# lbarseghyan/diffusion-models

Hardware: AMD Instinct MI355X
Metric: sampled images/sec, 32x32 U-Net (dim 64, mults 1-2-4-8), DDPM-1000 (higher is better)
Workload: dtype f32; 1 GPU; ddpm1000_32x32_unet64_b256_per_gpu; sampler=p_sample_loop (DDPM), sampler_steps=1000, batch_per_gpu=256, global_batch=256, hip_graph=True, graph_captures=1, parallelism=batch-shard x1, one all-gather per sample()

## Files before the change

### diffusion-models_amd/csrc/linattn_fused.hip

```cpp
#include "conv_device.h"

#include <cmath>
#include <vector>

namespace dm {

static constexpr int LA_DH = 32;
static constexpr int LA_HEADS = 4;
static constexpr int LA_HID = LA_DH * LA_HEADS;
static constexpr int LA_CTX = LA_DH * LA_DH + LA_DH;
static constexpr int LA_TOK1 = 128;
__host__ __device__ constexpr int la_tok1(int C) { return C <= 64 ? 256 : LA_TOK1; }
static constexpr int LA_TOK2 = 64;
static constexpr int LA_TOKI = 128;

__host__ __device__ static inline int la_row_of(int e, int half) { return (e & 3) + 8 * (e >> 2) + 4 * half; }

bool linattn_fused_eligible(int C, int heads, int dh) {
    static const bool off = env_flag("DM_NO_FUSED_LINATTN");
    return !off && heads == LA_HEADS && dh == LA_DH && (C == 64 || C == 128);
}

bool linattn_fused_pack(const float* w_qkv, const float* norm_g, const float* w_out, const float* mem_kv, int C,
                        std::vector<float>& wq, std::vector<float>& wk, std::vector<float>& wv, std::vector<float>& wo,
                        std::vector<float>& kbound) {
    const int G = C / 8;
    const float sq = std::sqrt((float)C);
    auto pack_proj = [&](int which, std::vector<float>& dst) {
        dst.assign((size_t)LA_HEADS * G * 64 * 4, 0.f);
        for (int h = 0; h < LA_HEADS; ++h)
            for (int g = 0; g < G; ++g)
                for (int lane = 0; lane < 64; ++lane)
                    for (int s = 0; s < 4; ++s) {
                        const int l = lane & 31, half = lane >> 5;
                        const int row = which * LA_HID + h * LA_DH + l, c = 8 * g + 4 * half + s;
                        dst[(((size_t)h * G + g) * 64 + lane) * 4 + s] = w_qkv[(size_t)row * C + c] * (norm_g[c] * sq);
                    }
    };
    pack_proj(0, wq);
    pack_proj(1, wk);
    pack_proj(2, wv);
    wo.clear();
    (void)w_out;
    kbound.assign(LA_HID, 0.f);
    bool ok = true;
    for (int h = 0; h < LA_HEADS; ++h)
        for (int d = 0; d < LA_DH; ++d) {
            double ss = 0;
            for (int c = 0; c < C; ++c) {
                const double v = (double)w_qkv[(size_t)(LA_HID + h * LA_DH + d) * C + c] * norm_g[c] * sq;
                ss += v * v;
            }
            float bnd = (float)(std::sqrt(ss) * 1.0001);
            for (int j = 0; j < 4; ++j) bnd = std::fmax(bnd, mem_kv[((size_t)h * LA_DH + d) * 4 + j]);
            kbound[h * LA_DH + d] = bnd;
            if (!(bnd < 40.f)) ok = false;
        }
    return ok;
}

size_t linattn_fused_ws_floats(int B, int n) {
    const int nblk = (n + LA_TOK1 - 1) / LA_TOK1;
    return (size_t)B * nblk * LA_HEADS * LA_CTX + (size_t)B * LA_HEADS * 128 * LA_DH;
}

template <int C, int TOK>
__device__ __forceinline__ void la_stage_rows(const float* __restrict__ xb, int nt, float* xs, float* rn) {
    constexpr int XS = C + 4, Q = C / 4;
    const int tid = threadIdx.x;
#pragma unroll
    for (int i = 0; i < TOK * Q / 256; ++i) {
        const int it = tid + 256 * i;
        const int row = it / Q, q = it - row * Q;
        f32x4 v = make_f32x4(0.f, 0.f, 0.f, 0.f);
        if (row < nt) v = *reinterpret_cast<const f32x4*>(xb + (size_t)row * C + 4 * q);
        *reinterpret_cast<f32x4*>(xs + row * XS + 4 * q) = v;
    }
    __syncthreads();
    if (tid < TOK) {
        float ss = 0.f;
#pragma unroll
        for (int q = 0; q < Q; ++q) {
            const f32x4 v = *reinterpret_cast<const f32x4*>(xs + tid * XS + 4 * q);
            ss += v.x * v.x + v.y * v.y + v.z * v.z + v.w * v.w;
        }
        rn[tid] = 1.0f / fmaxf(sqrtf(ss), 1e-12f);
    }
}

template <int C, int TOK>
__global__ __launch_bounds__(256) void linattn_ctx_fused_kernel(const float* __restrict__ x, const LinAttnFused w,
                                                                float* __restrict__ ws, int n, int nblk) {
    constexpr int G = C / 8, XS = C + 4;
    extern __shared__ __attribute__((aligned(16))) float smem[];
    float* xs = smem;
    float* rn = smem + TOK * XS;
    const int blk = blockIdx.x, b = blockIdx.y;
    const int tid = threadIdx.x, lane = tid & 63, h = tid >> 6;
    const int l31 = lane & 31, lh = lane >> 5;
    const int t0 = blk * TOK;
    const int nt = min(TOK, n - t0);

    f32x4 wk[G], wv[G];
#pragma unroll
    for (int g = 0; g < G; ++g) {
        wk[g] = *reinterpret_cast<const f32x4*>(w.wk + (((size_t)h * G + g) * 64 + lane) * 4);
        wv[g] = *reinterpret_cast<const f32x4*>(w.wv + (((size_t)h * G + g) * 64 + lane) * 4);
    }
    const float kb = w.kbound[h * LA_DH + l31];
    la_stage_rows<C, TOK>(x + ((size_t)b * n + t0) * C, nt, xs, rn);
    __syncthreads();

    f32x16 cacc;
#pragma unroll
    for (int e = 0; e < 16; ++e) cacc[e] = 0.f;
    float ksum = 0.f;
    if (blk == 0) {
        const float* mk = w.mem_kv + (size_t)h * LA_DH * 4;
        const float* mv = w.mem_kv + (size_t)(LA_HEADS + h) * LA_DH * 4;
#pragma unroll
        for (int j = 0; j < 4; j += 2) {
            const float a = __expf(mk[l31 * 4 + j + lh] - kb);
            ksum += a;
            cacc = __builtin_amdgcn_mfma_f32_32x32x2f32(a, mv[l31 * 4 + j + lh], cacc, 0, 0, 0);
        }
    }
    for (int st = 0; st < TOK / 32; ++st) {
        if (st * 32 >= nt) break;
        f32x16 kacc, vacc;
#pragma unroll
        for (int e = 0; e < 16; ++e) {
            kacc[e] = 0.f;
            vacc[e] = 0.f;
        }
        const float* xr = xs + (st * 32 + l31) * XS + 4 * lh;
#pragma unroll
        for (int g = 0; g < G; ++g) {
            const f32x4 a = *reinterpret_cast<const f32x4*>(xr + 8 * g);
#pragma unroll
            for (int s = 0; s < 4; ++s) {
                kacc = __builtin_amdgcn_mfma_f32_32x32x2f32(a[s], wk[g][s], kacc, 0, 0, 0);
                vacc = __builtin_amdgcn_mfma_f32_32x32x2f32(a[s], wv[g][s], vacc, 0, 0, 0);
            }
        }
#pragma unroll
        for (int m = 0; m < 4; ++m) {
            const f32x4 r4 = *reinterpret_cast<const f32x4*>(rn + st * 32 + 8 * m + 4 * lh);
#pragma unroll
            for (int i = 0; i < 4; ++i) {
                const int e = 4 * m + i;
                const bool valid = st * 32 + 8 * m + 4 * lh + i < nt;
                const float a = valid ? __expf(kacc[e] * r4[i] - kb) : 0.f;
                ksum += a;
                cacc = __builtin_amdgcn_mfma_f32_32x32x2f32(a, vacc[e] * r4[i], cacc, 0, 0, 0);
            }
        }
    }
    float* cp = ws + (((size_t)b * nblk + blk) * LA_HEADS + h) * LA_CTX;
#pragma unroll
    for (int e = 0; e < 16; ++e) cp[la_row_of(e, lh) * LA_DH + l31] = cacc[e];
    ksum += __shfl_xor(ksum, 32);
    if (lh == 0) cp[LA_DH * LA_DH + l31] = ksum;
}

template <int C>
__global__ __launch_bounds__(256) void linattn_ctx_reduce_kernel(const float* __restrict__ ws,
                                                                 const float* __restrict__ w_out,
                                                                 float* __restrict__ mz, int nblk) {
    constexpr int MT = C / 32;
    __shared__ float cs[LA_DH][LA_DH + 1];
    const int h = blockIdx.x, b = blockIdx.y;
    const int tid = threadIdx.x, lane = tid & 63, e4 = tid >> 6;
    const int l31 = lane & 31, lh = lane >> 5;
#pragma unroll
    for (int i = 0; i < 4; ++i) {
        const int d = 8 * e4 + 4 * lh + i;
        float c = 0.f, k = 0.f;
#pragma unroll 8
        for (int kb = 0; kb < nblk; ++kb) {
            const float* cp = ws + (((size_t)b * nblk + kb) * LA_HEADS + h) * LA_CTX;
            c += cp[d * LA_DH + l31];
            k += cp[LA_DH * LA_DH + d];
        }
        cs[d][l31] = c / k;
    }
    __syncthreads();
    const int mt = e4;
    if (mt < MT) {
        const float* wr = w_out + (size_t)(32 * mt + l31) * LA_HID + h * LA_DH;
        f32x16 acc;
#pragma unroll
        for (int e = 0; e < 16; ++e) acc[e] = 0.f;
#pragma unroll
        for (int st = 0; st < 16; ++st)
            acc = __builtin_amdgcn_mfma_f32_32x32x2f32(cs[l31][2 * st + lh], wr[2 * st + lh], acc, 0, 0, 0);
        float* op = mz + ((((size_t)b * LA_HEADS + h) * MT + mt) * 4) * 64 * 4 + lane * 4;
#pragma unroll
        for (int q = 0; q < 4; ++q)
            *reinterpret_cast<f32x4*>(op + q * 64 * 4) = make_f32x4(acc[4 * q], acc[4 * q + 1], acc[4 * q + 2], acc[4 * q + 3]);
    }
}

template <int C>
__device__ __forceinline__ void la_image_load(const float* __restrict__ xb, int t0, int n,
                                              f32x4 (&pre)[LA_TOKI * (C / 4) / 512]) {
    constexpr int Q = C / 4;
    const int tid = threadIdx.x;
#pragma unroll
    for (int i = 0; i < LA_TOKI * Q / 512; ++i) {
        const int it = tid + 512 * i;
        const int row = it / Q, q = it - row * Q;
        const int t = t0 + row;
        const f32x4 v = *reinterpret_cast<const f32x4*>(xb + (size_t)min(t, n - 1) * C + 4 * q);
        pre[i] = t < n ? v : make_f32x4(0.f, 0.f, 0.f, 0.f);
    }
}

template <int C>
__device__ __forceinline__ void la_image_store(const f32x4 (&pre)[LA_TOKI * (C / 4) / 512], float* xs, float* rn) {
    constexpr int XS = C + 4, Q = C / 4;
    const int tid = threadIdx.x;
#pragma unroll
    for (int i = 0; i < LA_TOKI * Q / 512; ++i) {
        const int it = tid + 512 * i;
        const int row = it / Q, q = it - row * Q;
        const f32x4 v = pre[i];
        *reinterpret_cast<f32x4*>(xs + row * XS + 4 * q) = v;
        float ss = v.x * v.x + v.y * v.y + v.z * v.z + v.w * v.w;
#pragma unroll
        for (int o = 1; o < Q; o <<= 1) ss += __shfl_xor(ss, o);
        if (q == 0) rn[row] = 1.0f / fmaxf(sqrtf(ss), 1e-12f);
    }
}

template <int C>
__global__ __launch_bounds__(512) void linattn_ctx_image_kernel(const float* __restrict__ x, const LinAttnFused w,
                                                                float* __restrict__ mz, int n) {
    constexpr int G = C / 8, XS = C + 4, CT = C / 32, TB = LA_TOKI, NP = TB * (C / 4) / 512;
    extern __shared__ __attribute__((aligned(16))) float smem[];
    float* rnb = smem + 2 * TB * XS;
    const int b = blockIdx.x;
    const int tid = threadIdx.x, lane = tid & 63, wid = tid >> 6;
    const int h = wid & 3, th = wid >> 2;
    const int l31 = lane & 31, lh = lane >> 5;
    const float* xb = x + (size_t)b * n * C;
    const int nb = (n + TB - 1) / TB;

    f32x4 wk[G];
#pragma unroll
    for (int g = 0; g < G; ++g) wk[g] = *reinterpret_cast<const f32x4*>(w.wk + (((size_t)h * G + g) * 64 + lane) * 4);
    const float kb = w.kbound[h * LA_DH + l31];

    f32x4 pre[NP];
    la_image_load<C>(xb, 0, n, pre);
    la_image_store<C>(pre, smem, rnb);
    __syncthreads();

    f32x16 pacc[CT];
#pragma unroll
    for (int ct = 0; ct < CT; ++ct)
#pragma unroll
        for (int e = 0; e < 16; ++e) pacc[ct][e] = 0.f;
    float ksum = 0.f;
    for (int blk = 0; blk < nb; ++blk) {
        const bool more = blk + 1 < nb;
        if (more) la_image_load<C>(xb, (blk + 1) * TB, n, pre);
        const float* xs = smem + (blk & 1) * TB * XS;
        const float* rn = rnb + (blk & 1) * TB;
#pragma unroll
        for (int j = 0; j < 2; ++j) {
            const int tb = 32 * (th + 2 * j);
            const int nt = n - blk * TB - tb;
            if (nt <= 0) break;
            f32x16 kacc;
#pragma unroll
            for (int e = 0; e < 16; ++e) kacc[e] = 0.f;
            const float* xr = xs + (tb + l31) * XS + 4 * lh;
#pragma unroll
            for (int g = 0; g < G; ++g) {
                const f32x4 a = *reinterpret_cast<const f32x4*>(xr + 8 * g);
#pragma unroll
                for (int s = 0; s < 4; ++s) kacc = __builtin_amdgcn_mfma_f32_32x32x2f32(a[s], wk[g][s], kacc, 0, 0, 0);
            }
            const float* xc = xs + (tb + 4 * lh) * XS + l31;
#pragma unroll
            for (int m = 0; m < 4; ++m) {
                const f32x4 r4 = *reinterpret_cast<const f32x4*>(rn + tb + 8 * m + 4 * lh);
#pragma unroll
                for (int i = 0; i < 4; ++i) {
                    const int e = 4 * m + i;
                    const bool valid = 8 * m + 4 * lh + i < nt;
                    const float a = valid ? __expf(kacc[e] * r4[i] - kb) : 0.f;
                    ksum += a;
                    const float ar = a * r4[i];
#pragma unroll
                    for (int ct = 0; ct < CT; ++ct)
                        pacc[ct] = __builtin_amdgcn_mfma_f32_32x32x2f32(xc[(8 * m + i) * XS + 32 * ct], ar, pacc[ct], 0, 0, 0);
                }
            }
        }
        if (more) la_image_store<C>(pre, smem + ((blk + 1) & 1) * TB * XS, rnb + ((blk + 1) & 1) * TB);
        __syncthreads();
    }

    float* cps = smem + (size_t)h * CT * 16 * 64 + lane;
    float* cks = smem + LA_HEADS * CT * 16 * 64 + h * 64 + lane;
    if (th == 1) {
#pragma unroll
        for (int ct = 0; ct < CT; ++ct)
#pragma unroll
            for (int e = 0; e < 16; ++e) cps[(ct * 16 + e) * 64] = pacc[ct][e];
        *cks = ksum;
    }
    __syncthreads();
    if (th == 1) return;

    ksum += *cks;
    f32x16 tacc;
#pragma unroll
    for (int e = 0; e < 16; ++e) tacc[e] = 0.f;
    {
        const float* mk = w.mem_kv + (size_t)h * LA_DH * 4;
        const float* mv = w.mem_kv + (size_t)(LA_HEADS + h) * LA_DH * 4;
#pragma unroll
        for (int j = 0; j < 4; j += 2) {
            const float a = __expf(mk[l31 * 4 + j + lh] - kb);
            ksum += a;
            tacc = __builtin_amdgcn_mfma_f32_32x32x2f32(mv[l31 * 4 + j + lh], a, tacc, 0, 0, 0);
        }
    }
#pragma unroll
    for (int ct = 0; ct < CT; ++ct)
#pragma unroll
        for (int q = 0; q < 4; ++q) {
            const f32x4 wv = *reinterpret_cast<const f32x4*>(w.wv + (((size_t)h * G + 4 * ct + q) * 64 + lane) * 4);
#pragma unroll
            for (int i = 0; i < 4; ++i) {
                const int e = 4 * q + i;
                tacc = __builtin_amdgcn_mfma_f32_32x32x2f32(wv[i], pacc[ct][e] + cps[(ct * 16 + e) * 64], tacc, 0, 0, 0);
            }
        }
    ksum += __shfl_xor(ksum, 32);
#pragma unroll
    for (int e = 0; e < 16; ++e) tacc[e] = tacc[e] / ksum;
#pragma unroll
    for (int mt = 0; mt < CT; ++mt) {
        const float* wr = w.wo_raw + (size_t)(32 * mt + l31) * LA_HID + h * LA_DH + 4 * lh;
        f32x16 macc;
#pragma unroll
        for (int e = 0; e < 16; ++e) macc[e] = 0.f;
#pragma unroll
        for (int q = 0; q < 4; ++q) {
            const f32x4 wo = *reinterpret_cast<const f32x4*>(wr + 8 * q);
#pragma unroll
            for (int i = 0; i < 4; ++i) macc = __builtin_amdgcn_mfma_f32_32x32x2f32(tacc[4 * q + i], wo[i], macc, 0, 0, 0);
        }
        float* op = mz + ((((size_t)b * LA_HEADS + h) * CT + mt) * 4) * 64 * 4 + lane * 4;
#pragma unroll
        for (int q = 0; q < 4; ++q)
            *reinterpret_cast<f32x4*>(op + q * 64 * 4) =
                make_f32x4(macc[4 * q], macc[4 * q + 1], macc[4 * q + 2], macc[4 * q + 3]);
    }
}

template <int C>
__global__ __launch_bounds__(256) void linattn_out_fused_kernel(const float* __restrict__ x, const LinAttnFused w,
                                                                const float* __restrict__ mz, float* __restrict__ y,
                                                                int n, int add_x, float scale) {
    constexpr int G = C / 8, XS = C + 4, TOK = LA_TOK2, MT = C / 32, Q = C / 4;
    extern __shared__ __attribute__((aligned(16))) float smem[];
    float* xs = smem;
    float* rn = smem + TOK * XS;
    float* zb = rn + TOK;
    const int blk = blockIdx.x, b = blockIdx.y;
    const int tid = threadIdx.x, lane = tid & 63, h = tid >> 6;
    const int l31 = lane & 31, lh = lane >> 5;
    const int t0 = blk * TOK;
    const int nt = min(TOK, n - t0);

    f32x4 wq[G];
#pragma unroll
    for (int g = 0; g < G; ++g) wq[g] = *reinterpret_cast<const f32x4*>(w.wq + (((size_t)h * G + g) * 64 + lane) * 4);
    f32x4 mreg[MT][4];
    {
        const float* mzp = mz + ((size_t)b * LA_HEADS + h) * MT * 4 * 64 * 4 + lane * 4;
#pragma unroll
        for (int mt = 0; mt < MT; ++mt)
#pragma unroll
            for (int e4 = 0; e4 < 4; ++e4) mreg[mt][e4] = *reinterpret_cast<const f32x4*>(mzp + (mt * 4 + e4) * 64 * 4);
    }
    la_stage_rows<C, TOK>(x + ((size_t)b * n + t0) * C, nt, xs, rn);
    __syncthreads();

    for (int st = 0; st < TOK / 32; ++st) {
        if (st * 32 >= nt) break;
        f32x16 qacc;
#pragma unroll
        for (int e = 0; e < 16; ++e) qacc[e] = 0.f;
        const float* xr = xs + (st * 32 + l31) * XS + 4 * lh;
#pragma unroll
        for (int g = 0; g < G; ++g) {
            const f32x4 a = *reinterpret_cast<const f32x4*>(xr + 8 * g);
#pragma unroll
            for (int s = 0; s < 4; ++s) qacc = __builtin_amdgcn_mfma_f32_32x32x2f32(wq[g][s], a[s], qacc, 0, 0, 0);
        }
        const float r = rn[st * 32 + l31];
        float m = -INFINITY;
#pragma unroll
        for (int e = 0; e < 16; ++e) {
            qacc[e] *= r;
            m = fmaxf(m, qacc[e]);
        }
        m = fmaxf(m, __shfl_xor(m, 32));
        float ssum = 0.f;
#pragma unroll
        for (int e = 0; e < 16; ++e) {
            qacc[e] = __expf(qacc[e] - m);
            ssum += qacc[e];
        }
        ssum += __shfl_xor(ssum, 32);
        const float inv = scale / ssum;
#pragma unroll
        for (int e = 0; e < 16; ++e) qacc[e] *= inv;
#pragma unroll
        for (int mt = 0; mt < MT; ++mt) {
            f32x16 zacc;
#pragma unroll
            for (int e = 0; e < 16; ++e) zacc[e] = 0.f;
#pragma unroll
            for (int e4 = 0; e4 < 4; ++e4) {
#pragma unroll
                for (int i = 0; i < 4; ++i)
                    zacc = __builtin_amdgcn_mfma_f32_32x32x2f32(mreg[mt][e4][i], qacc[4 * e4 + i], zacc, 0, 0, 0);
            }
            float* zr = zb + (h * 32 + l31) * XS + 32 * mt + 4 * lh;
#pragma unroll
            for (int m4 = 0; m4 < 4; ++m4)
                *reinterpret_cast<f32x4*>(zr + 8 * m4) =
                    make_f32x4(zacc[4 * m4], zacc[4 * m4 + 1], zacc[4 * m4 + 2], zacc[4 * m4 + 3]);
        }
        __syncthreads();
#pragma unroll
        for (int i = 0; i < 32 * Q / 256; ++i) {
            const int it = tid + 256 * i;
            const int tok = it / Q, q4 = it - tok * Q;
            f32x4 z = *reinterpret_cast<const f32x4*>(w.bias + 4 * q4);
#pragma unroll
            for (int hh = 0; hh < LA_HEADS; ++hh) z += *reinterpret_cast<const f32x4*>(zb + (hh * 32 + tok) * XS + 4 * q4);
            float ss = z.x * z.x + z.y * z.y + z.z * z.z + z.w * z.w;
#pragma unroll
            for (int o = 1; o < Q; o <<= 1) ss += __shfl_xor(ss, o);
            z = z * fast_rsq(fmaxf(ss, 1e-24f)) * *reinterpret_cast<const f32x4*>(w.og + 4 * q4);
            if (add_x) z += *reinterpret_cast<const f32x4*>(xs + (st * 32 + tok) * XS + 4 * q4);
            if (st * 32 + tok < nt)
                *reinterpret_cast<f32x4*>(y + ((size_t)b * n + t0 + st * 32 + tok) * C + 4 * q4) = z;
        }
        __syncthreads();
    }
}

template <int C, int TOK1>
static int launch_ctx(const LinAttnFused& w, const float* x, float* ws, int B, int n, int nblk, hipStream_t s) {
    const size_t lds1 = (size_t)(TOK1 * (C + 4) + TOK1) * 4;
    static LdsOptIn lds_flag;
    if (lds_opt_in(lds_flag, reinterpret_cast<const void*>(linattn_ctx_fused_kernel<C, TOK1>), 1)) return 1;
    hipLaunchKernelGGL((linattn_ctx_fused_kernel<C, TOK1>), dim3(nblk, B), dim3(256), lds1, s, x, w, ws, n, nblk);
    DM_CHECK_HIP(hipGetLastError());
    return 0;
}

static bool la_image_form(int B, int n, int C) { return B >= 256 && (C == 64 || n > 64); }

template <int C>
static int launch_ctx_image(const LinAttnFused& w, const float* x, float* mz, int B, int n, hipStream_t s) {
    const size_t lds = (size_t)(2 * LA_TOKI * (C + 4) + 2 * LA_TOKI) * 4;
    static LdsOptIn lds_flag;
    if (lds_opt_in(lds_flag, reinterpret_cast<const void*>(linattn_ctx_image_kernel<C>), 1)) return 1;
    hipLaunchKernelGGL(linattn_ctx_image_kernel<C>, dim3(B), dim3(512), lds, s, x, w, mz, n);
    DM_CHECK_HIP(hipGetLastError());
    return 0;
}

template <int C>
static int launch_c(const LinAttnFused& w, const float* x, float* ws, float* y, int B, int n, bool add_x, hipStream_t s) {
    const bool image = la_image_form(B, n, C);
    const bool big = la_tok1(C) == 256 && (size_t)B * ((n + 255) / 256) >= 512;
    const int tok1 = big ? 256 : LA_TOK1;
    const int nblk = image ? 0 : (n + tok1 - 1) / tok1;
    const size_t lds2 = (size_t)(LA_TOK2 * (C + 4) + LA_TOK2 + LA_HEADS * 32 * (C + 4)) * 4;
    static LdsOptIn lds_flag;
    if (lds_opt_in(lds_flag, reinterpret_cast<const void*>(linattn_out_fused_kernel<C>), 1)) return 1;
    const bool timed = prof::enabled();
    const double tokens = (double)B * n;
    float* ctxn = ws + (size_t)B * nblk * LA_HEADS * LA_CTX;
    if (image) {
        if (timed && prof::begin("linattn_ctx_image_kernel",
                                 2.0 * tokens * (2.0 * LA_HID * C) + (double)B * 2.0 * (2.0 * LA_HID * LA_DH * C),
                                 4.0 * tokens * C, s))
            return 1;
        if (launch_ctx_image<C>(w, x, ctxn, B, n, s)) return 1;
        if (timed && prof::end(s)) return 1;
    } else {
        if (timed && prof::begin("linattn_ctx_fused_kernel", 2.0 * tokens * (2.0 * LA_HID * C + LA_HID * LA_DH),
                                 4.0 * tokens * C, s))
            return 1;
        if (big ? launch_ctx<C, (C <= 64 ? 256 : LA_TOK1)>(w, x, ws, B, n, nblk, s)
                : launch_ctx<C, LA_TOK1>(w, x, ws, B, n, nblk, s))
            return 1;
        if (timed && prof::end(s)) return 1;
        if (timed && prof::begin("linattn_ctx_reduce_kernel", (double)B * 2.0 * LA_HID * LA_DH * C,
                                 4.0 * B * ((double)nblk * LA_HEADS * LA_CTX + LA_HID * C + LA_HID * C), s))
            return 1;
        hipLaunchKernelGGL(linattn_ctx_reduce_kernel<C>, dim3(LA_HEADS, B), dim3(256), 0, s, ws, w.wo_raw, ctxn, nblk);
        DM_CHECK_HIP(hipGetLastError());
        if (timed && prof::end(s)) return 1;
    }
    if (timed && prof::begin("linattn_out_fused_kernel", 2.0 * tokens * (2.0 * LA_HID * C + LA_HID * LA_DH),
                             8.0 * tokens * C, s))
        return 1;
    hipLaunchKernelGGL(linattn_out_fused_kernel<C>, dim3((n + LA_TOK2 - 1) / LA_TOK2, B), dim3(256), lds2, s, x, w,
                       ctxn, y, n, add_x ? 1 : 0, 1.0f / sqrtf((float)LA_DH));
    DM_CHECK_HIP(hipGetLastError());
    if (timed && prof::end(s)) return 1;
    return 0;
}

int launch_linattn_fused(const LinAttnFused& w, const float* x, float* ws, float* y, int B, int n, bool add_x,
                         hipStream_t s) {
    DM_REQUIRE(w.C == 64 || w.C == 128, "fused LinearAttention: C must be 64 or 128");
    if (w.C == 64) return launch_c<64>(w, x, ws, y, B, n, add_x, s);
    return launch_c<128>(w, x, ws, y, B, n, add_x, s);
}

}
```

Baseline: 58.19 images/s.

## Add persistent head-summing output kernel for fused linear attention

Adds a new output kernel for linear attention that processes multiple token windows per workgroup with double-buffered prefetch of the input. It folds the head context into the output projection (precomputed mz held in registers), so each token tile needs one MFMA chain summed over heads instead of per-head context products. Row sums of squares use DPP lane reductions. It is selected for batch >= 32, which covers the default path. It adds a large LDS footprint and register pressure, which can reduce occupancy.

Result: faster. 58.89 images/s, median of 6 (+1.2%).

```diff
diff --git a/diffusion-models_amd/csrc/linattn_fused.hip b/diffusion-models_amd/csrc/linattn_fused.hip
--- a/diffusion-models_amd/csrc/linattn_fused.hip
+++ b/diffusion-models_amd/csrc/linattn_fused.hip
@@ -1,6 +1,7 @@
 #include "conv_device.h"
 
 #include <cmath>
+#include <type_traits>
 #include <vector>
 
 namespace dm {
@@ -201,14 +202,14 @@
     }
 }
 
-template <int C>
+template <int C, int TOK = LA_TOKI, int NT = 512>
 __device__ __forceinline__ void la_image_load(const float* __restrict__ xb, int t0, int n,
-                                              f32x4 (&pre)[LA_TOKI * (C / 4) / 512]) {
+                                              f32x4 (&pre)[TOK * (C / 4) / NT]) {
     constexpr int Q = C / 4;
     const int tid = threadIdx.x;
 #pragma unroll
-    for (int i = 0; i < LA_TOKI * Q / 512; ++i) {
-        const int it = tid + 512 * i;
+    for (int i = 0; i < TOK * Q / NT; ++i) {
+        const int it = tid + NT * i;
         const int row = it / Q, q = it - row * Q;
         const int t = t0 + row;
         const f32x4 v = *reinterpret_cast<const f32x4*>(xb + (size_t)min(t, n - 1) * C + 4 * q);
@@ -216,13 +217,49 @@
     }
 }
 
-template <int C>
-__device__ __forceinline__ void la_image_store(const f32x4 (&pre)[LA_TOKI * (C / 4) / 512], float* xs, float* rn) {
-    constexpr int XS = C + 4, Q = C / 4;
+template <int CTRL, int N>
+__device__ __forceinline__ void la_dpp_add(float (&v)[N]) {
+#pragma unroll
+    for (int i = 0; i < N; ++i)
+        v[i] += __builtin_bit_cast(float, __builtin_amdgcn_update_dpp(0, __builtin_bit_cast(int, v[i]), CTRL, 0xF, 0xF, false));
+}
+template <int Q, int N>
+__device__ __forceinline__ void la_row_sums(float (&v)[N]) {
+    static_assert(Q == 16 || Q == 32, "a row is 16 or 32 lanes");
+    la_dpp_add<0xB1>(v);
+    la_dpp_add<0x4E>(v);
+    la_dpp_add<0x141>(v);
+    la_dpp_add<0x140>(v);
+    if (Q == 32) {
+#pragma unroll
+        for (int i = 0; i < N; ++i) v[i] += __shfl_xor(v[i], 16);
+    }
+}
+
+template <int C, int TOK = LA_TOKI, int NT = 512, bool SS = false>
+__device__ __forceinline__ void la_image_store(const f32x4 (&pre)[TOK * (C / 4) / NT], float* xs, float* rn) {
+    constexpr int XS = C + 4, Q = C / 4, N = TOK * Q / NT;
     const int tid = threadIdx.x;
-#pragma unroll
-    for (int i = 0; i < LA_TOKI * Q / 512; ++i) {
-        const int it = tid + 512 * i;
+    if (SS) {
+        float ss[N];
+#pragma unroll
+        for (int i = 0; i < N; ++i) {
+            const int it = tid + NT * i;
+            const int row = it / Q, q = it - row * Q;
+            const f32x4 v = pre[i];
+            *reinterpret_cast<f32x4*>(xs + row * XS + 4 * q) = v;
+            ss[i] = v.x * v.x + v.y * v.y + v.z * v.z + v.w * v.w;
+        }
+        la_row_sums<Q>(ss);
+        if (tid % Q == 0) {
+#pragma unroll
+            for (int i = 0; i < N; ++i) rn[(tid + NT * i) / Q] = ss[i];
+        }
+        return;
+    }
+#pragma unroll
+    for (int i = 0; i < N; ++i) {
+        const int it = tid + NT * i;
         const int row = it / Q, q = it - row * Q;
         const f32x4 v = pre[i];
         *reinterpret_cast<f32x4*>(xs + row * XS + 4 * q) = v;
@@ -459,6 +496,161 @@
     }
 }
 
+static constexpr int LA_OUTW = 4096;
+
+template <int C>
+__global__ __launch_bounds__(256, 2) void linattn_out_headsum_kernel(const float* __restrict__ x, const LinAttnFused w,
+                                                                     const float* __restrict__ mz,
+                                                                     float* __restrict__ y, int n, int run, int add_x,
+                                                                     float scale) {
+    constexpr int G = C / 8, XS = C + 4, MT = C / 32, Q = C / 4, TW = LA_OUTW / C, TILES = TW / 32, NP = TW * Q / 256;
+    constexpr int PB = LA_HEADS * TILES * 16 * 64;
+    constexpr bool ZALIAS = C == 64;
+    static_assert(!ZALIAS || TW * XS <= PB, "z does not fit over p");
+    extern __shared__ __attribute__((aligned(16))) float smem[];
+    float* rnb = smem + 2 * TW * XS;
+    float* pb = rnb + 2 * TW;
+    float* zb = ZALIAS ? pb : pb + PB;
+    float* ssb = (ZALIAS ? pb + PB : zb + TW * XS);
+    const int b = blockIdx.y;
+    const int tid = threadIdx.x, lane = tid & 63, wv = tid >> 6;
+    const int l31 = lane & 31, lh = lane >> 5;
+    const int mt = ZALIAS ? (wv & 1) : wv, zt = ZALIAS ? (wv >> 1) : 0;
+    const float* xb = x + (size_t)b * n * C;
+    const int nw = (n + TW - 1) / TW;
+    const int w0 = blockIdx.x * run, w1 = min(nw, w0 + run);
+
+    f32x4 wq[G];
+#pragma unroll
+    for (int g = 0; g < G; ++g) wq[g] = *reinterpret_cast<const f32x4*>(w.wq + (((size_t)wv * G + g) * 64 + lane) * 4);
+    f32x4 mreg[LA_HEADS][4];
+#pragma unroll
+    for (int hh = 0; hh < LA_HEADS; ++hh)
+#pragma unroll
+        for (int e4 = 0; e4 < 4; ++e4)
+            mreg[hh][e4] = *reinterpret_cast<const f32x4*>(
+                mz + ((((size_t)b * LA_HEADS + hh) * MT + mt) * 4 + e4) * 64 * 4 + lane * 4);
+    f32x16 bias;
+#pragma unroll
+    for (int m4 = 0; m4 < 4; ++m4) {
+        const f32x4 v = *reinterpret_cast<const f32x4*>(w.bias + 32 * mt + 8 * m4 + 4 * lh);
+#pragma unroll
+        for (int i = 0; i < 4; ++i) bias[4 * m4 + i] = v[i];
+    }
+    const int q4 = tid & (Q - 1);
+    const f32x4 og = *reinterpret_cast<const f32x4*>(w.og + 4 * q4);
+
+    f32x4 pre[NP];
+    la_image_load<C, TW, 256>(xb, w0 * TW, n, pre);
+    la_image_store<C, TW, 256, true>(pre, smem, rnb);
+    __syncthreads();
+
+    for (int wi = w0; wi < w1; ++wi) {
+        const bool more = wi + 1 < w1;
+        if (more) {
+            if ((wi + 2) * TW <= n) {
+                const float* xw = xb + ((size_t)(wi + 1) * TW + tid / Q) * C + 4 * q4;
+#pragma unroll
+                for (int i = 0; i < NP; ++i) pre[i] = *reinterpret_cast<const f32x4*>(xw + (size_t)i * (256 / Q) * C);
+            } else {
+                la_image_load<C, TW, 256>(xb, (wi + 1) * TW, n, pre);
+            }
+        }
+        const int buf = (wi - w0) & 1;
+        const float* xs = smem + buf * TW * XS;
+        const float* rn = rnb + buf * TW;
+        const int t0 = wi * TW;
+        const int nt = min(TW, n - t0);
+
+#pragma unroll
+        for (int st = 0; st < TILES; ++st) {
+            if (st * 32 >= nt) break;
+            f32x16 qacc;
+#pragma unroll
+            for (int e = 0; e < 16; ++e) qacc[e] = 0.f;
+            const float* xr = xs + (st * 32 + l31) * XS + 4 * lh;
+#pragma unroll
+            for (int g = 0; g < G; ++g) {
+                const f32x4 a = *reinterpret_cast<const f32x4*>(xr + 8 * g);
+#pragma unroll
+                for (int s = 0; s < 4; ++s) qacc = __builtin_amdgcn_mfma_f32_32x32x2f32(wq[g][s], a[s], qacc, 0, 0, 0);
+            }
+            const float r = 1.0f / fmaxf(sqrtf(rn[st * 32 + l31]), 1e-12f);
+            float m = -INFINITY;
+#pragma unroll
+            for (int e = 0; e < 16; ++e) m = fmaxf(m, qacc[e]);
+            m = fmaxf(m, __shfl_xor(m, 32));
+            m *= r;
+            float ssum = 0.f;
+#pragma unroll
+            for (int e = 0; e < 16; ++e) {
+                qacc[e] = __expf(qacc[e] * r - m);
+                ssum += qacc[e];
+            }
+            ssum += __shfl_xor(ssum, 32);
+            const float inv = scale / ssum;
+            float* pw = pb + (size_t)(wv * TILES + st) * 16 * 64 + lane * 4;
+#pragma unroll
+            for (int e4 = 0; e4 < 4; ++e4)
+                *reinterpret_cast<f32x4*>(pw + e4 * 64 * 4) = make_f32x4(qacc[4 * e4] * inv, qacc[4 * e4 + 1] * inv,
+                                                                          qacc[4 * e4 + 2] * inv, qacc[4 * e4 + 3] * inv);
+        }
+        __syncthreads();
+
+        const bool live = zt * 32 < nt;
+        f32x16 zacc;
+        float ss = 0.f;
+        if (live) {
+            zacc = bias;
+#pragma unroll
+            for (int hh = 0; hh < LA_HEADS; ++hh) {
+                const float* pr = pb + (size_t)(hh * TILES + zt) * 16 * 64 + lane * 4;
+#pragma unroll
+                for (int e4 = 0; e4 < 4; ++e4) {
+                    const f32x4 p = *reinterpret_cast<const f32x4*>(pr + e4 * 64 * 4);
+#pragma unroll
+                    for (int i = 0; i < 4; ++i)
+                        zacc = __builtin_amdgcn_mfma_f32_32x32x2f32(mreg[hh][e4][i], p[i], zacc, 0, 0, 0);
+                }
+            }
+#pragma unroll
+            for (int e = 0; e < 16; ++e) ss = fmaf(zacc[e], zacc[e], ss);
+            ss += __shfl_xor(ss, 32);
+        }
+        if (ZALIAS) __syncthreads();
+        if (live) {
+            float* zr = zb + (zt * 32 + l31) * XS + 32 * mt + 4 * lh;
+#pragma unroll
+            for (int m4 = 0; m4 < 4; ++m4)
+                *reinterpret_cast<f32x4*>(zr + 8 * m4) =
+                    make_f32x4(zacc[4 * m4], zacc[4 * m4 + 1], zacc[4 * m4 + 2], zacc[4 * m4 + 3]);
+            if (lh == 0) ssb[mt * TW + zt * 32 + l31] = ss;
+        }
+        __syncthreads();
+
+        auto rows_out = [&](auto whole) {
+            float* yw = y + ((size_t)b * n + t0 + tid / Q) * C + 4 * q4;
+#pragma unroll
+            for (int i = 0; i < NP; ++i) {
+                const int tok = tid / Q + i * (256 / Q);
+                if (whole.value || tok < nt) {
+                    f32x4 z = *reinterpret_cast<const f32x4*>(zb + tok * XS + 4 * q4);
+                    float sq = ssb[tok];
+#pragma unroll
+                    for (int m = 1; m < MT; ++m) sq += ssb[m * TW + tok];
+                    z = z * fast_rsq(fmaxf(sq, 1e-24f)) * og;
+                    if (add_x) z += *reinterpret_cast<const f32x4*>(xs + tok * XS + 4 * q4);
+                    *reinterpret_cast<f32x4*>(yw + (size_t)i * (256 / Q) * C) = z;
+                }
+            }
+        };
+        if (nt == TW) rows_out(std::true_type{});
+        else rows_out(std::false_type{});
+        if (more) la_image_store<C, TW, 256, true>(pre, smem + (buf ^ 1) * TW * XS, rnb + (buf ^ 1) * TW);
+        __syncthreads();
+    }
+}
+
 template <int C, int TOK1>
 static int launch_ctx(const LinAttnFused& w, const float* x, float* ws, int B, int n, int nblk, hipStream_t s) {
     const size_t lds1 = (size_t)(TOK1 * (C + 4) + TOK1) * 4;
@@ -477,6 +669,33 @@
     static LdsOptIn lds_flag;
     if (lds_opt_in(lds_flag, reinterpret_cast<const void*>(linattn_ctx_image_kernel<C>), 1)) return 1;
     hipLaunchKernelGGL(linattn_ctx_image_kernel<C>, dim3(B), dim3(512), lds, s, x, w, mz, n);
+    DM_CHECK_HIP(hipGetLastError());
+    return 0;
+}
+
+static constexpr int LA_OUT_WGS = 512;
+static bool la_out_headsum_form(int B, int n, int C) {
+#ifdef DM_LA_OUT_FORM
+    return DM_LA_OUT_FORM;
+#else
+    return B >= 32;
+#endif
+}
+
+template <int C>
+static int launch_out_headsum(const LinAttnFused& w, const float* x, const float* mz, float* y, int B, int n, bool add_x,
+                              hipStream_t s) {
+    constexpr int TW = LA_OUTW / C, TILES = TW / 32;
+    constexpr bool ZALIAS = C == 64;
+    const size_t lds = (size_t)(2 * TW * (C + 4) + 2 * TW + LA_HEADS * TILES * 16 * 64 + (ZALIAS ? 0 : TW * (C + 4)) +
+                                (C / 32) * TW) * 4;
+    static LdsOptIn lds_flag;
+    if (lds_opt_in(lds_flag, reinterpret_cast<const void*>(linattn_out_headsum_kernel<C>), 1)) return 1;
+    const int nw = (n + TW - 1) / TW;
+    const int per_image = std::min(nw, std::max(1, (LA_OUT_WGS + B - 1) / B));
+    const int run = (nw + per_image - 1) / per_image;
+    hipLaunchKernelGGL(linattn_out_headsum_kernel<C>, dim3((nw + run - 1) / run, B), dim3(256), lds, s, x, w, mz, y, n,
+                       run, add_x ? 1 : 0, 1.0f / sqrtf((float)LA_DH));
     DM_CHECK_HIP(hipGetLastError());
     return 0;
 }
@@ -515,12 +734,17 @@
         DM_CHECK_HIP(hipGetLastError());
         if (timed && prof::end(s)) return 1;
     }
-    if (timed && prof::begin("linattn_out_fused_kernel", 2.0 * tokens * (2.0 * LA_HID * C + LA_HID * LA_DH),
-                             8.0 * tokens * C, s))
+    const bool headsum = la_out_headsum_form(B, n, C);
+    if (timed && prof::begin(headsum ? "linattn_out_headsum_kernel" : "linattn_out_fused_kernel",
+                             2.0 * tokens * (2.0 * LA_HID * C + LA_HID * LA_DH), 8.0 * tokens * C, s))
         return 1;
-    hipLaunchKernelGGL(linattn_out_fused_kernel<C>, dim3((n + LA_TOK2 - 1) / LA_TOK2, B), dim3(256), lds2, s, x, w,
-                       ctxn, y, n, add_x ? 1 : 0, 1.0f / sqrtf((float)LA_DH));
-    DM_CHECK_HIP(hipGetLastError());
+    if (headsum) {
+        if (launch_out_headsum<C>(w, x, ctxn, y, B, n, add_x, s)) return 1;
+    } else {
+        hipLaunchKernelGGL(linattn_out_fused_kernel<C>, dim3((n + LA_TOK2 - 1) / LA_TOK2, B), dim3(256), lds2, s, x, w,
+                           ctxn, y, n, add_x ? 1 : 0, 1.0f / sqrtf((float)LA_DH));
+        DM_CHECK_HIP(hipGetLastError());
+    }
     if (timed && prof::end(s)) return 1;
     return 0;
 }
```
